# sunnyHelen/JPerceiver

Hardware: AMD Instinct MI355X
Metric: train images/sec (full train step, synthetic 3-frame batches) (higher is better)
Workload: dtype f32

## Files before the change

### include/jperceiver_hip.h

```cpp
#ifndef JPERCEIVER_HIP_H
#define JPERCEIVER_HIP_H
#include <stdint.h>

#ifdef __cplusplus
extern "C" {
#endif

int jp_conv2d_fwd(const float* x, const float* w, const float* bias, float* y, int N, int Cin, int H, int W, int Cout, int KH, int stride, int pad, int pad_mode, int act, float* ws, int ws_state, float* split_ws, const float* amax_x, float* amax_y, int* amax_y_done, float* amax_ws, float* bn_stats, int* bn_stats_parts, void* stream);
int jp_conv2d_fwd_src3(const float* x0, int c0, int up0, const float* x1, int c1, int up1, const float* x2, int c2, int up2, const float* w, const float* bias, float* y, int N, int H, int W, int Cout, int KH, int stride, int pad, int pad_mode, int act, float* ws, int ws_state, float* split_ws, const float* amax_x0, const float* amax_x1, const float* amax_x2, float* amax_y, int* amax_y_done, float* amax_ws, float* bn_stats, int* bn_stats_parts, void* stream);
int jp_conv2d_dgrad(const float* dy, const float* w, float* dx, int N, int Cin, int H, int W, int Cout, int KH, int stride, int pad, int pad_mode, int accumulate, float* ws, int ws_state, float* split_ws, const float* amax_dy, float* amax_dx, int* amax_dx_done, float* amax_ws, void* stream);
int jp_conv2d_dgrad_src3(const float* dy, const float* w, float* dx0, int c0, int up0, int acc0, float* dx1, int c1, int up1, int acc1, float* dx2, int c2, int up2, int acc2, int N, int H, int W, int Cout, int KH, int stride, int pad, int pad_mode, float* ws, int ws_state, float* split_ws, const float* amax_dy, float* amax_dx0, int* amax_dx0_done, float* amax_ws, void* stream);
long jp_conv2d_dgrad_src3_split_floats(int c0, int up0, int c1, int up1, int c2, int up2, int N, int H, int W);
int jp_conv2d_dgrad_src3_ok(int c0, int up0, int c1, int up1, int c2, int up2, int N, int H, int W, int Cout, int KH, int stride, int pad, int pad_mode);
int jp_conv2d_up_head_ok(int c0, int up0, int c1, int c2, int Cout, int KH, int stride, int pad, int pad_mode, int H, int W);
int jp_conv2d_wgrad(const float* x, const float* dy, float* dw, int N, int Cin, int H, int W, int Cout, int KH, int stride, int pad, int pad_mode, int accumulate, float* ws, long ws_floats, const float* amax_x, const float* amax_dy, float* amax_ws, void* stream);
int jp_conv2d_wgrad_src3(const float* x0, int c0, int up0, const float* x1, int c1, int up1, const float* x2, int c2, int up2, const float* dy, float* dw, int N, int H, int W, int Cout, int KH, int stride, int pad, int pad_mode, int accumulate, float* ws, long ws_floats, const float* amax_x0, const float* amax_x1, const float* amax_x2, const float* amax_dy, float* amax_ws, void* stream);
long jp_conv2d_ws_floats(int Cin, int Cout, int KH, int which);
long jp_conv2d_fwd_bn_stats_floats(int N, int OH, int OW, int Cout);
long jp_conv2d_fwd_split_floats(int N, int Cin, int H, int W, int Cout, int KH, int stride, int pad);
long jp_conv2d_dgrad_split_floats(int N, int Cin, int H, int W, int Cout, int KH, int stride, int pad);
long jp_conv2d_wgrad_ws_floats(int N, int Cin, int H, int W, int Cout, int KH, int stride, int pad);
long jp_conv2d_wgrad_src3_ws_floats(int c0, int up0, int c1, int up1, int c2, int up2, int N, int H, int W, int Cout, int KH, int stride, int pad, int pad_mode);
long jp_channel_sum_ws_floats(int N, int C, int HW);
int jp_channel_sum(const float* x, float* out, int N, int C, int HW, int accumulate, float* ws, void* stream);
int jp_pack_job_bytes(void);
int jp_pack_record_begin(void* host_jobs, int max_jobs);
int jp_pack_record_end(void);
int jp_pack_mode_is_split(int mode);
int jp_pack_replay(const void* jobs, int njobs, long total_elems, long generic_elems, void* stream);

int jp_amax_slot_floats(void);
int jp_conv2d_amax_ws_floats(void);
int jp_amax(const float* x, long n, float* out, void* stream);
int jp_amax_into(const float* x, long n, float* out, void* stream);
int jp_split_scheme(void);

long jp_bn_ws_doubles(int N, int C, int HW);
int jp_bn_train_fwd(const float* x, const float* gamma, const float* beta, const float* residual, float* y, float* running_mean, float* running_var, float* save_mean, float* save_invstd, double* ws, int N, int C, int HW, float momentum, float eps, int relu, int n_updates, float* amax_y, const float* conv_stats, int conv_parts, void* stream);
int jp_bn_train_bwd(const float* dy, const float* x, const float* y, const float* gamma, const float* beta, const float* save_mean, const float* save_invstd, float* dx, float* dres, float* dgamma, float* dbeta, double* ws, int N, int C, int HW, int relu, int acc_param_grads, float* amax_dx, void* stream);
int jp_bn_eval_fwd(const float* x, const float* gamma, const float* beta, const float* running_mean, const float* running_var, const float* residual, float* y, int N, int C, int HW, float eps, int relu, void* stream);
int jp_bn_relu_pool_fwd(const float* x, const float* gamma, const float* beta, float* pooled, uint8_t* idx, float* running_mean, float* running_var, float* save_mean, float* save_invstd, double* ws, int N, int C, int H, int W, float momentum, float eps, int n_updates, float* amax_y, void* stream);
long jp_bn_relu_pool_bwd_ws_doubles(int N, int C, int H, int W);
int jp_bn_relu_pool_bwd(const float* dpool, const uint8_t* idx, const float* x, const float* gamma, const float* beta, const float* save_mean, const float* save_invstd, float* dx, float* dgamma, float* dbeta, double* ws, int N, int C, int H, int W, int acc_param_grads, void* stream);

int jp_bn_fold_conv(const float* w, const float* conv_bias, const float* gamma, const float* beta, const float* running_mean, const float* running_var, float eps, float* w_out, float* bias_out, int Cout, int K, void* stream);
int jp_add_relu(const float* a, const float* b, float* out, long n, int relu, float* amax_out, void* stream);

int jp_maxpool_fwd(const float* x, float* y, uint8_t* idx, int NC, int H, int W, int k, int s, int p, void* stream);
int jp_maxpool_bwd(const float* dy, const uint8_t* idx, float* dx, const float* addend, int NC, int H, int W, int k, int s, int p, float* amax_dx, void* stream);
int jp_upsample2x_fwd(const float* x, float* y, int N, int C, int H, int W, int dstC, int dc0, void* stream);
int jp_upsample2x_bwd(const float* dy, float* dx, int N, int C, int H, int W, int Ctot, int c0, int accumulate, void* stream);
int jp_copy_channels(const float* src, float* dst, int N, int C, int HW, int srcC, int sc0, int dstC, int dc0, int accumulate, void* stream);
int jp_axpby(const float* a, const float* b, float* out, long n, float alpha, float beta, void* stream);
int jp_sum_n(const float* a0, const float* a1, const float* a2, const float* a3, const float* a4, float* out, long n, float* amax_out, void* stream);
int jp_mul(const float* a, const float* b, float* out, long n, float scale, void* stream);
int jp_affine(const float* a, float* out, long n, float scale, float shift, void* stream);
int jp_act_fwd(const float* x, float* y, long n, int act, void* stream);
int jp_act_bwd(const float* dy, const float* y, float* dx, long n, int act, float* amax_dx, void* stream);
long jp_act_bwd_bias_ws_floats(int N, int C, int HW);
int jp_act_bwd_bias(const float* dy, const float* y, float* dx, float* dbias, int N, int C, int HW, int act, float* amax_dx, float* bias_ws, void* stream);
int jp_mul_bcast_c(const float* a, const float* s, float* out, int N, int C, int HW, void* stream);
int jp_mul_bcast_c_bwd_s(const float* dout, const float* a, float* ds, int N, int C, int HW, void* stream);
int jp_bilinear_fwd(const float* x, float* y, int NC, int H, int W, int OH, int OW, void* stream);
int jp_bilinear_bwd(const float* dy, float* dx, int NC, int H, int W, int OH, int OW, int accumulate, void* stream);
int jp_area_downsample(const float* x, float* y, int NC, int H, int W, int f, void* stream);
int jp_fill(float* out, long n, float v, void* stream);
int jp_warp_perspective(const float* src, const float* Hm, float* dst, int B, int h, int w, int OH, int OW, void* stream);
int jp_softmax_c2(const float* x, float* y, int N, int HW, void* stream);
int jp_disp_to_depth(const float* disp, float* depth, long n, float min_depth, float max_depth, void* stream);
int jp_scale_label_assemble(const float* zwarp, const float* laywarp, const uint8_t* polymask, float* out, int B, int H, int W, int mode, void* stream);
int jp_fill_convex_poly(const int* pts, int npts, uint8_t* mask, int H, int W, void* stream);

int jp_gemm_strided_batched(const float* A, const float* B, float* C, int M, int N, int K, int lda, int ldb, int ldc, long strideA, long strideB, long strideC, int batch, int transA, int transB, float alpha, float beta, void* stream);
int jp_bias_act_rows(float* y, const float* bias, int M, int N, int act, void* stream);
int jp_colsum(const float* x, float* out, int M, int N, int accumulate, void* stream);
int jp_colmax(const float* E, float* val, int64_t* arg, int B, int R, int Cn, void* stream);
int jp_colmax_bwd(const float* dval, const int64_t* arg, float* dE, int B, int R, int Cn, void* stream);
int jp_gather_cols(const float* V, const int64_t* arg, float* T, int B, int C, int Nn, void* stream);
int jp_gather_cols_bwd(const float* dT, const int64_t* arg, float* dV, int B, int C, int Nn, void* stream);
int jp_spatial_mean(const float* x, float* out, int BC, int HW, float scale, void* stream);
int jp_spatial_mean_bwd(const float* dout, float* dx, int BC, int HW, float scale, void* stream);
int jp_bcast_matmul_fwd(const float* attn, const float* V, float* out, int B, int C, int n, void* stream);
int jp_bcast_matmul_bwd(const float* attn, const float* V, const float* dOut, float* dattn, float* dV, int B, int C, int n, void* stream);
int jp_ratio_finalize(const double* acc, float* out, double scale, void* stream);

int jp_pose_fwd(const float* axisangle, const float* translation, const float* K, float* T, float* P, int B, int invert, void* stream);
int jp_pose_bwd(const double* dP, const float* axisangle, const float* translation, const float* K, float* daxisangle, float* dtranslation, int B, int invert, int accumulate, void* stream);
int jp_cgt_warp_fwd(const float* disp, int hs, int ws, const float* invK, const float* P, const float* color, float* pred, int B, int H, int W, float min_depth, float max_depth, void* stream);
int jp_cgt_warp_bwd(const float* dpred, const float* disp, int hs, int ws, const float* invK, const float* P, const float* color, float* ddisp_up, double* dP, int B, int H, int W, float min_depth, float max_depth, int accumulate, void* stream);
int jp_ssim_l1_fwd(const float* pred, const float* target, float* out, int B, int H, int W, void* stream);
int jp_ssim_l1_bwd(const float* pred, const float* target, const int64_t* min_index, int cand, const float* gout, float gscale, float* dpred, int B, int H, int W, void* stream);
int jp_minreproj_fwd(const float* c0, const float* c1, const float* c2, const float* c3, const float* noise0, const float* noise1, int64_t* min_index, double* acc, long total, void* stream);
int jp_scalar_finalize(const double* in, float* out, int n, double scale, void* stream);
int jp_ssim_map(const float* x, const float* y, float* out, int NC, int H, int W, void* stream);
int jp_backproject(const float* depth, const float* invK, float* out, int B, int H, int W, void* stream);
int jp_project(const float* points, const float* K, const float* T, float* out, int B, int H, int W, float eps, void* stream);

int jp_row_sum(const float* x, double* out, int rows, int cols, void* stream);
int jp_smooth_fwd(const float* disp, const double* dsum, const float* img, double* acc, int B, int h, int w, void* stream);
int jp_smooth_bwd(const float* disp, const double* dsum, const float* img, const float* gout, float scale, float* g, double* gd, float* ddisp, int B, int h, int w, int accumulate, void* stream);
int jp_scale_loss_fwd(const float* disp, int hs, int ws, const float* label, double* acc, int B, int FH, int FW, float min_depth, float max_depth, int y_lo, int y_hi, int x_lo, int x_hi, void* stream);
int jp_scale_loss_bwd(const float* disp, int hs, int ws, const float* label, const double* acc, const float* gout, float scale, float* ddisp, int B, int FH, int FW, float min_depth, float max_depth, int y_lo, int y_hi, int x_lo, int x_hi, int accumulate, void* stream);
int jp_layout_loss_fwd(const float* logits, const float* label, const float* sdf, double* sums, float* loss, int B, int h, int w, float w0, float w1, float lw, float cew, float l2w, float ra, float ralpha, float rbeta, void* stream);
int jp_layout_loss_bwd(const float* logits, const float* label, const float* sdf, const double* sums, const float* gout, float* dlogits, int B, int h, int w, float w0, float w1, float lw, float cew, float l2w, float ra, float ralpha, float rbeta, int accumulate, void* stream);
int jp_sdf(const float* label, float* sdf, int* ws, int B, int h, int w, void* stream);
int jp_l1_fwd(const float* a, const float* b, double* acc, long n, void* stream);
int jp_l1_bwd(const float* a, const float* b, const float* gout, float scale, float* da, float* db, long n, void* stream);

int jp_sumsq_blocks(void);
int jp_grad_sumsq_partials(const float* g, double* partials, long n, void* stream);
int jp_sum_doubles(const double* in, double* out, int count, void* stream);
int jp_adam_clip_step(float* p, const float* g, float* m, float* v, long n, const double* normsq, float grad_scale, float max_norm, double lr, double beta1, double beta2, double eps, int step, void* stream);
int jp_adam_clip_step_dev(float* p, const float* g, float* m, float* v, long n, const double* normsq, float grad_scale, float max_norm, double beta1, double beta2, double eps, const float* state, void* stream);
int jp_rng_keep_mask(float* out, long n, uint64_t seed, float p_drop, void* stream);
int jp_rng_normal(float* out, long n, uint64_t seed, void* stream);
int jp_rng_keep_mask_dev(float* out, long n, const long* base, long offset, float p_drop, void* stream);
int jp_rng_normal_dev(float* out, long n, const long* base, long offset, void* stream);

int jp_confusion2(const float* logits, const float* gt, double* counts, int B, int HW, void* stream);
int jp_depth_eval_prepare(const float* disp_resized, const float* gt, float* pred, uint8_t* valid, int H, int W, int y0, int y1, int x0, int x1, float dmin, float dmax, void* stream);
// ... 67 lines not shown
```

### jperceiver_amd/csrc/bn.hip

```cpp
#include "jp_common.h"
#include <algorithm>

namespace {

constexpr int TPB = 256;

__global__ __launch_bounds__(TPB) void bn_stats_kernel(const float* __restrict__ x, double* __restrict__ sums,
                                                       int C, int HW, int CH, int chunk) {
    __shared__ double sm[4];
    const int c = blockIdx.x;
    const int n = blockIdx.y / CH, ck = blockIdx.y - n * CH;
    const int beg = ck * chunk, end = min(HW, beg + chunk);
    const float* xp = x + ((size_t)n * C + c) * HW;
    double s = 0.0, q = 0.0;
    float fs = 0.f, fq = 0.f;
    int run = 0;
    if (((HW | chunk) & 3) == 0) {
        const float4* x4 = reinterpret_cast<const float4*>(xp);
        for (int i = (beg >> 2) + threadIdx.x; i < (end >> 2); i += TPB) {
            const float4 v = x4[i];
            fs += (v.x + v.y) + (v.z + v.w);
            fq += (v.x * v.x + v.y * v.y) + (v.z * v.z + v.w * v.w);
            if (++run == 8) { s += fs; q += fq; fs = fq = 0.f; run = 0; }
        }
    } else {
        for (int i = beg + threadIdx.x; i < end; i += TPB) {
            const float v = xp[i];
            fs += v;
            fq += v * v;
            if (++run == 32) { s += fs; q += fq; fs = fq = 0.f; run = 0; }
        }
    }
    s += fs; q += fq;
    s = jp_block_sum_d(s, sm);
    q = jp_block_sum_d(q, sm);
    if (threadIdx.x == 0) {
        sums[(size_t)(2 * c) * gridDim.y + blockIdx.y] = s;
        sums[(size_t)(2 * c + 1) * gridDim.y + blockIdx.y] = q;
    }
}

__global__ __launch_bounds__(TPB) void bn_stats_fold_kernel(const float* __restrict__ conv_stats, double* __restrict__ sums, int parts,
                                                            int p0, int np) {
    __shared__ double sm[4];
    const int c = blockIdx.x;
    const float* a = conv_stats + ((size_t)c * 2 + 0) * parts + p0;
    const float* b = conv_stats + ((size_t)c * 2 + 1) * parts + p0;
    double s = 0.0, q = 0.0;
    for (int i = threadIdx.x; i < np; i += TPB) { s += (double)a[i]; q += (double)b[i]; }
    s = jp_block_sum_d(s, sm);
    q = jp_block_sum_d(q, sm);
    if (threadIdx.x == 0) { sums[2 * c] = s; sums[2 * c + 1] = q; }
}

__device__ __forceinline__ void bn_channel_stats(const double* __restrict__ sums, int c, int S, double count, float eps,
                                                 double* __restrict__ tot , float* mean_out, float* invstd_out,
                                                 double* var_out) {
    if (threadIdx.x < 64) {
        double a = 0.0, b = 0.0;
        for (int i = threadIdx.x; i < S; i += 64) {
            a += sums[(size_t)(2 * c) * S + i];
            b += sums[(size_t)(2 * c + 1) * S + i];
        }
        a = jp_wave_sum_d(a);
        b = jp_wave_sum_d(b);
        if (threadIdx.x == 0) { tot[0] = a; tot[1] = b; }
    }
    __syncthreads();
    const double m = tot[0] / count;
    double var = tot[1] / count - m * m;
    if (var < 0.0) var = 0.0;
    *mean_out = (float)m;
    *invstd_out = (float)(1.0 / sqrt(var + (double)eps));
    *var_out = var;
}

__device__ __forceinline__ float bn_affine(float x, float sc, float sh) { return fmaf(x, sc, sh); }
__device__ __forceinline__ float bn_shift(float beta, float mean, float sc) { return fmaf(-mean, sc, beta); }

__device__ __forceinline__ void bn_apply_body(const float* __restrict__ x, const float* __restrict__ residual,
                                              float* __restrict__ y, float sc, float sh, size_t base, int HW, int relu,
                                              unsigned* __restrict__ amax = nullptr) {
    float mx = 0.f;
    if ((HW & 3) == 0) {
        const float4* x4 = reinterpret_cast<const float4*>(x + base);
        const float4* r4 = residual ? reinterpret_cast<const float4*>(residual + base) : nullptr;
        float4* y4 = reinterpret_cast<float4*>(y + base);
        for (int i = blockIdx.x * TPB + threadIdx.x; i < (HW >> 2); i += gridDim.x * TPB) {
            const float4 a = x4[i];
            float4 v = make_float4(bn_affine(a.x, sc, sh), bn_affine(a.y, sc, sh), bn_affine(a.z, sc, sh), bn_affine(a.w, sc, sh));
            if (r4) { const float4 r = r4[i]; v.x += r.x; v.y += r.y; v.z += r.z; v.w += r.w; }
            if (relu) { v.x = fmaxf(v.x, 0.f); v.y = fmaxf(v.y, 0.f); v.z = fmaxf(v.z, 0.f); v.w = fmaxf(v.w, 0.f); }
            y4[i] = v;
            mx = fmaxf(fmaxf(mx, fmaxf(jp_fmag(v.x), jp_fmag(v.y))), fmaxf(jp_fmag(v.z), jp_fmag(v.w)));
        }
    } else {
        for (int i = blockIdx.x * TPB + threadIdx.x; i < HW; i += gridDim.x * TPB) {
            float v = bn_affine(x[base + i], sc, sh);
            if (residual) v += residual[base + i];
            if (relu) v = fmaxf(v, 0.f);
            y[base + i] = v;
            mx = fmaxf(mx, jp_fmag(v));
        }
    }
    jp_block_amax_commit(mx, amax);
}

__global__ __launch_bounds__(TPB) void bn_apply_kernel(const float* __restrict__ x, const double* __restrict__ sums,
                                                       float* __restrict__ save_mean, float* __restrict__ save_invstd,
                                                       float* __restrict__ running_mean, float* __restrict__ running_var,
                                                       const float* __restrict__ gamma,
                                                       const float* __restrict__ beta,
                                                       const float* __restrict__ residual, float* __restrict__ y,
                                                       int C, int HW, int relu, double count, float momentum, float eps,
                                                       int n_updates, int S, unsigned* __restrict__ amax) {
    __shared__ double tot[2];
    const int nc = blockIdx.y;
    const int c = nc % C;
    float mean, invstd;
    double var;
    bn_channel_stats(sums, c, S, count, eps, tot, &mean, &invstd, &var);
    if (nc < C && blockIdx.x == 0 && threadIdx.x == 0) {
        save_mean[c] = mean;
        save_invstd[c] = invstd;
        if (running_mean) {
            const float unb = (float)(count > 1.0 ? var * count / (count - 1.0) : var);
            float rm = running_mean[c], rv = running_var[c];
            for (int i = 0; i < n_updates; ++i) {
                rm = (1.f - momentum) * rm + momentum * mean;
                rv = (1.f - momentum) * rv + momentum * unb;
            }
            running_mean[c] = rm;
            running_var[c] = rv;
        }
    }
    const float sc = invstd * gamma[c];
    const float sh = bn_shift(beta[c], mean, sc);
    bn_apply_body(x, residual, y, sc, sh, (size_t)nc * HW, HW, relu, amax);
}

__global__ __launch_bounds__(TPB) void bn_eval_kernel(const float* __restrict__ x, const float* __restrict__ rm,
                                                      const float* __restrict__ rv, const float* __restrict__ gamma,
                                                      const float* __restrict__ beta,
                                                      const float* __restrict__ residual, float* __restrict__ y,
                                                      int C, int HW, float eps, int relu) {
    const int nc = blockIdx.y;
    const int c = nc % C;
    const float sc = gamma[c] / sqrtf(rv[c] + eps);
    const float sh = bn_shift(beta[c], rm[c], sc);
    bn_apply_body(x, residual, y, sc, sh, (size_t)nc * HW, HW, relu);
}

__global__ __launch_bounds__(TPB) void bn_bwd_reduce_kernel(const float* __restrict__ dy,
                                                            const float* __restrict__ x,
                                                            const float* __restrict__ y,
                                                            const float* __restrict__ mean,
                                                            const float* __restrict__ invstd,
// ... 35 lines not shown
            if (++run == 32) { s += fs; q += fq; fs = fq = 0.f; run = 0; }
        }
    }
#undef JP_BN_RED1
    s += fs; q += fq;
    s = jp_block_sum_d(s, sm);
    q = jp_block_sum_d(q, sm);
    if (threadIdx.x == 0) {
        sums[(size_t)(2 * c) * gridDim.y + blockIdx.y] = s;
        sums[(size_t)(2 * c + 1) * gridDim.y + blockIdx.y] = q;
    }
}

__global__ __launch_bounds__(TPB) void bn_bwd_apply_kernel(const float* __restrict__ dy, const float* __restrict__ x,
                                                           const float* __restrict__ y,
                                                           const float* __restrict__ mean,
                                                           const float* __restrict__ invstd,
                                                           const float* __restrict__ gamma,
                                                           const float* __restrict__ beta,
                                                           const double* __restrict__ sums, float* __restrict__ dx,
                                                           float* __restrict__ dres, float* __restrict__ dgamma,
                                                           float* __restrict__ dbeta, int C, int HW, double count,
                                                           int relu, int acc_param_grads, int S, unsigned* __restrict__ amax) {
    float mx = 0.f;
    const int nc = blockIdx.y;
    const int c = nc % C;
    const float mu = mean[c], is = invstd[c], g = gamma[c];
    const float sc = is * g, sh = bn_shift(beta[c], mu, sc);
    __shared__ double tot[2];
    if (threadIdx.x < 64) {
        double a = 0.0, b = 0.0;
        for (int i = threadIdx.x; i < S; i += 64) {
            a += sums[(size_t)(2 * c) * S + i];
            b += sums[(size_t)(2 * c + 1) * S + i];
        }
        a = jp_wave_sum_d(a);
        b = jp_wave_sum_d(b);
        if (threadIdx.x == 0) { tot[0] = a; tot[1] = b; }
    }
    __syncthreads();
    const double t1 = tot[0], t2 = tot[1];
    const float k1 = (float)(t1 / count), k2 = (float)(t2 / count);
    if (nc < C && blockIdx.x == 0 && threadIdx.x == 0) {
        const float dg = (float)t2, db = (float)t1;
        dgamma[c] = acc_param_grads ? dgamma[c] + dg : dg;
        dbeta[c] = acc_param_grads ? dbeta[c] + db : db;
    }
    const size_t base = (size_t)nc * HW;
    const float gi = g * is;
#define JP_BN_APP1(D, X, Yv, OUT, RES)                                     \
    {                                                                      \
        float d_ = (D);                                                    \
        if (relu && !((y ? (Yv) : bn_affine((X), sc, sh)) > 0.f)) d_ = 0.f; \
        RES = d_;                                                          \
        OUT = gi * (d_ - k1 - ((X) - mu) * is * k2);                       \
    }
    if ((HW & 3) == 0) {
        const float4* d4 = reinterpret_cast<const float4*>(dy + base);
        const float4* x4 = reinterpret_cast<const float4*>(x + base);
        const float4* y4 = y ? reinterpret_cast<const float4*>(y + base) : nullptr;
        float4* o4 = reinterpret_cast<float4*>(dx + base);
        float4* r4 = dres ? reinterpret_cast<float4*>(dres + base) : nullptr;
        for (int i = blockIdx.x * TPB + threadIdx.x; i < (HW >> 2); i += gridDim.x * TPB) {
            const float4 d = d4[i], a = x4[i];
            const float4 yy = y4 ? y4[i] : make_float4(0.f, 0.f, 0.f, 0.f);
            float4 o, r;
            JP_BN_APP1(d.x, a.x, yy.x, o.x, r.x) JP_BN_APP1(d.y, a.y, yy.y, o.y, r.y)
            JP_BN_APP1(d.z, a.z, yy.z, o.z, r.z) JP_BN_APP1(d.w, a.w, yy.w, o.w, r.w)
            o4[i] = o;
            mx = fmaxf(fmaxf(mx, fmaxf(jp_fmag(o.x), jp_fmag(o.y))), fmaxf(jp_fmag(o.z), jp_fmag(o.w)));
            if (r4) r4[i] = r;
        }
    } else {
        for (int i = blockIdx.x * TPB + threadIdx.x; i < HW; i += gridDim.x * TPB) {
            float o, r;
            JP_BN_APP1(dy[base + i], x[base + i], y[base + i], o, r)
            dx[base + i] = o;
            mx = fmaxf(mx, jp_fmag(o));
            if (dres) dres[base + i] = r;
        }
    }
    jp_block_amax_commit(mx, amax);
#undef JP_BN_APP1
}

__global__ __launch_bounds__(TPB) void channel_sum_kernel(const float* __restrict__ x, float* __restrict__ out,
                                                          int C, int HW, int CH, int chunk, float* __restrict__ part) {
    __shared__ double sm[4];
    const int c = blockIdx.x;
    const int n = blockIdx.y / CH, ck = blockIdx.y - n * CH;
    const int beg = ck * chunk, end = min(HW, beg + chunk);
    const float* xp = x + ((size_t)n * C + c) * HW;
    double s = 0.0;
    float fs = 0.f;
    int run = 0;
    for (int i = beg + threadIdx.x; i < end; i += TPB) {
        fs += xp[i];
        if (++run == 32) { s += fs; fs = 0.f; run = 0; }
    }
    s += fs;
    s = jp_block_sum_d(s, sm);
    if (threadIdx.x == 0) {
        if (part) part[(size_t)c * gridDim.y + blockIdx.y] = (float)s;
        else atomicAdd(&out[c], (float)s);
    }
}
__global__ void channel_fold_kernel(const float* __restrict__ part, float* __restrict__ out, int C, int S) {
    const int c = blockIdx.x * blockDim.x + threadIdx.x;
    if (c >= C) return;
    float s = 0.f;
    for (int i = 0; i < S; ++i) s += part[(size_t)c * S + i];
    out[c] += s;
}


constexpr int SP_TW = 64, SP_TH = 16;

__global__ __launch_bounds__(TPB) void bn_pool_fwd_kernel(const float* __restrict__ x, const double* __restrict__ sums,
                                                          float* __restrict__ save_mean, float* __restrict__ save_invstd,
                                                          float* __restrict__ running_mean, float* __restrict__ running_var,
                                                          const float* __restrict__ gamma, const float* __restrict__ beta,
                                                          float* __restrict__ y, uint8_t* __restrict__ idx, int C, int H, int W,
                                                          int OH, int OW, double count, float momentum, float eps, int n_updates,
                                                          int S, unsigned* __restrict__ amax) {
    constexpr int PW = (SP_TW - 1) * 2 + 3, PH = (SP_TH - 1) * 2 + 3;
    __shared__ float tile[PW * PH];
    __shared__ double tot[2];
    const int nc = blockIdx.z, c = nc % C;
    float mean, invstd;
    double var;
    bn_channel_stats(sums, c, S, count, eps, tot, &mean, &invstd, &var);
    if (nc < C && blockIdx.x == 0 && blockIdx.y == 0 && threadIdx.x == 0) {
        save_mean[c] = mean;
        save_invstd[c] = invstd;
        if (running_mean) {
            const float unb = (float)(count > 1.0 ? var * count / (count - 1.0) : var);
            float rm = running_mean[c], rv = running_var[c];
            for (int i = 0; i < n_updates; ++i) {
                rm = (1.f - momentum) * rm + momentum * mean;
                rv = (1.f - momentum) * rv + momentum * unb;
            }
            running_mean[c] = rm;
            running_var[c] = rv;
        }
    }
    const float sc = invstd * gamma[c], sh = bn_shift(beta[c], mean, sc);
    const float* xp = x + (size_t)nc * H * W;
    const int ox0 = blockIdx.x * SP_TW, oy0 = blockIdx.y * SP_TH;
    const int ix0 = ox0 * 2 - 1, iy0 = oy0 * 2 - 1;
    for (int i = threadIdx.x; i < PW * PH; i += TPB) {
        const int ly = i / PW, lx = i - ly * PW;
        const int iy = iy0 + ly, ix = ix0 + lx;
        tile[i] = ((unsigned)iy < (unsigned)H && (unsigned)ix < (unsigned)W) ? fmaxf(bn_affine(xp[iy * W + ix], sc, sh), 0.f) : -INFINITY;
    }
    __syncthreads();
    const int tx = threadIdx.x & 63, q = threadIdx.x >> 6;
    float best[4];
    int bi[4];
#pragma unroll
    for (int j = 0; j < 4; ++j) { best[j] = -INFINITY; bi[j] = 0; }
    const float* base = tile + (q * 4 * 2) * PW + tx * 2;
#pragma unroll
    for (int r = 0; r < 3 * 2 + 3; ++r) {
        float rv = base[r * PW];
        int rk = 0;
#pragma unroll
// ... 71 lines not shown
    for (int i = threadIdx.x; i < S; i += 64) {
        a += sums[(size_t)(2 * c) * S + i];
        b += sums[(size_t)(2 * c + 1) * S + i];
    }
    a = jp_wave_sum_d(a);
    b = jp_wave_sum_d(b);
    if (threadIdx.x == 0) {
        k12[2 * c] = (float)(a / count);
        k12[2 * c + 1] = (float)(b / count);
        dgamma[c] = acc_param_grads ? dgamma[c] + (float)b : (float)b;
        dbeta[c] = acc_param_grads ? dbeta[c] + (float)a : (float)a;
    }
}

__global__ __launch_bounds__(TPB) void bn_pool_bwd_apply_kernel(const float* __restrict__ dpool, const uint8_t* __restrict__ idx,
                                                                const float* __restrict__ x, const float* __restrict__ mean,
                                                                const float* __restrict__ invstd, const float* __restrict__ gamma,
                                                                const float* __restrict__ beta, const float* __restrict__ k12,
                                                                float* __restrict__ dx, long units, int C, int OH, int OW, int RB,
                                                                int bands) {
    const long u = (long)blockIdx.x * TPB + threadIdx.x;
    if (u >= units) return;
    const int OW2 = OW >> 1, W = 2 * OW;
    const int q = (int)(u % OW2);
    const long v = u / OW2;
    const int b = (int)(v % bands);
    const long nc = v / bands;
    const int c = (int)(nc % C);
    const float mu = mean[c], is = invstd[c], gm = gamma[c];
    const float sc = is * gm, sh = bn_shift(beta[c], mu, sc), gi = gm * is;
    const float k1 = k12[2 * c], k2 = k12[2 * c + 1];
    const int i0 = b * RB, i1 = min(OH, i0 + RB);
    const float* dp = dpool + nc * (long)OH * OW + 2 * q;
    const uint8_t* ip = idx + nc * (long)OH * OW + 2 * q;
    const float* xp = x + nc * 4L * OH * OW + 4 * q;
    float* op = dx + nc * 4L * OH * OW + 4 * q;
    const bool right = 2 * q + 2 < OW;
    float g[2][3];
    int k[2][3];
    auto load = [&](int slot, int i) {
        if (i < OH) {
            const float2 a = *reinterpret_cast<const float2*>(dp + (long)i * OW);
            const uchar2 cc = *reinterpret_cast<const uchar2*>(ip + (long)i * OW);
            g[slot][0] = a.x; g[slot][1] = a.y; k[slot][0] = cc.x; k[slot][1] = cc.y;
            g[slot][2] = right ? dp[(long)i * OW + 2] : 0.f;
            k[slot][2] = right ? (int)ip[(long)i * OW + 2] : -1;
        } else {
#pragma unroll
            for (int j = 0; j < 3; ++j) { g[slot][j] = 0.f; k[slot][j] = -1; }
        }
    };
    auto fin = [&](float d, float xv) {
        if (!(bn_affine(xv, sc, sh) > 0.f)) d = 0.f;
        return gi * (d - k1 - (xv - mu) * is * k2);
    };
    load(0, i0);
    for (int i = i0; i < i1; ++i) {
        load(1, i + 1);
        const float4 x0 = *reinterpret_cast<const float4*>(xp + (long)(2 * i) * W);
        const float4 x1 = *reinterpret_cast<const float4*>(xp + (long)(2 * i + 1) * W);
        float4 r0, r1;
        r0.x = k[0][0] == 4 ? g[0][0] : 0.f;
        r0.y = (k[0][0] == 5 ? g[0][0] : 0.f) + (k[0][1] == 3 ? g[0][1] : 0.f);
        r0.z = k[0][1] == 4 ? g[0][1] : 0.f;
        r0.w = (k[0][1] == 5 ? g[0][1] : 0.f) + (k[0][2] == 3 ? g[0][2] : 0.f);
        r1.x = (k[0][0] == 7 ? g[0][0] : 0.f) + (k[1][0] == 1 ? g[1][0] : 0.f);
        r1.y = (k[0][0] == 8 ? g[0][0] : 0.f) + (k[0][1] == 6 ? g[0][1] : 0.f) + (k[1][0] == 2 ? g[1][0] : 0.f) + (k[1][1] == 0 ? g[1][1] : 0.f);
        r1.z = (k[0][1] == 7 ? g[0][1] : 0.f) + (k[1][1] == 1 ? g[1][1] : 0.f);
        r1.w = (k[0][1] == 8 ? g[0][1] : 0.f) + (k[0][2] == 6 ? g[0][2] : 0.f) + (k[1][1] == 2 ? g[1][1] : 0.f) + (k[1][2] == 0 ? g[1][2] : 0.f);
        *reinterpret_cast<float4*>(op + (long)(2 * i) * W) = make_float4(fin(r0.x, x0.x), fin(r0.y, x0.y), fin(r0.z, x0.z), fin(r0.w, x0.w));
        *reinterpret_cast<float4*>(op + (long)(2 * i + 1) * W) = make_float4(fin(r1.x, x1.x), fin(r1.y, x1.y), fin(r1.z, x1.z), fin(r1.w, x1.w));
#pragma unroll
        for (int j = 0; j < 3; ++j) { g[0][j] = g[1][j]; k[0][j] = k[1][j]; }
    }
}

void chunking(int N, int C, int HW, int* CH, int* chunk) {
    int ch = std::max(1, 2048 / std::max(1, N * C));
    ch = std::min(ch, std::max(1, HW / 2048));
    *chunk = (HW + ch - 1) / ch;
    *CH = (HW + *chunk - 1) / *chunk;
}

}

extern "C" long jp_bn_ws_doubles(int N, int C, int HW) {
    int CH, chunk;
    chunking(N, C, HW, &CH, &chunk);
    return 2L * C * N * CH;
}

extern "C" int jp_bn_train_fwd(const float* x, const float* gamma, const float* beta, const float* residual,
                               float* y, float* running_mean, float* running_var, float* save_mean,
                               float* save_invstd, double* ws, int N, int C, int HW, float momentum, float eps,
                               int relu, int n_updates, float* amax_y, const float* conv_stats, int conv_parts, void* stream) {
    JP_CHECK_ARG(x && gamma && beta && y && save_mean && save_invstd && ws, "bn_train_fwd: null pointer");
    JP_CHECK_ARG(N > 0 && C > 0 && HW > 0, "bn_train_fwd: bad dims");
    hipStream_t st = (hipStream_t)stream;
    int CH, chunk;
    chunking(N, C, HW, &CH, &chunk);
    int S = N * CH;
    if (conv_stats && conv_parts > 0) {
        hipLaunchKernelGGL(bn_stats_fold_kernel, dim3(C), dim3(TPB), 0, st, conv_stats, ws, conv_parts, 0, conv_parts);
        S = 1;
    } else {
        hipLaunchKernelGGL(bn_stats_kernel, dim3(C, N * CH), dim3(TPB), 0, st, x, ws, C, HW, CH, chunk);
    }
    const int gx = std::min(jp_cdiv(HW, 4 * TPB), 64);
    hipLaunchKernelGGL(bn_apply_kernel, dim3(gx, N * C), dim3(TPB), 0, st, x, ws, save_mean, save_invstd, running_mean,
                       running_var, gamma, beta, residual, y, C, HW, relu, (double)N * HW, momentum, eps, n_updates, S,
                       reinterpret_cast<unsigned*>(amax_y));
    JP_LAUNCH_CHECK();
}

extern "C" int jp_bn_train_bwd(const float* dy, const float* x, const float* y, const float* gamma, const float* beta,
                               const float* save_mean, const float* save_invstd, float* dx, float* dres,
                               float* dgamma, float* dbeta, double* ws, int N, int C, int HW, int relu,
                               int acc_param_grads, float* amax_dx, void* stream) {
    JP_CHECK_ARG(dy && x && gamma && beta && save_mean && save_invstd && dx && dgamma && dbeta && ws, "bn_train_bwd: null pointer");
    hipStream_t st = (hipStream_t)stream;
    int CH, chunk;
    chunking(N, C, HW, &CH, &chunk);
    hipLaunchKernelGGL(bn_bwd_reduce_kernel, dim3(C, N * CH), dim3(TPB), 0, st, dy, x, y, save_mean, save_invstd, gamma,
                       beta, ws, C, HW, CH, chunk, relu);
    const int gx = std::min(jp_cdiv(HW, 4 * TPB), 64);
    hipLaunchKernelGGL(bn_bwd_apply_kernel, dim3(gx, N * C), dim3(TPB), 0, st, dy, x, y, save_mean, save_invstd, gamma,
                       beta, ws, dx, dres, dgamma, dbeta, C, HW, (double)N * HW, relu, acc_param_grads, N * CH,
                       reinterpret_cast<unsigned*>(amax_dx));
    JP_LAUNCH_CHECK();
}

extern "C" int jp_bn_relu_pool_fwd(const float* x, const float* gamma, const float* beta, float* pooled, uint8_t* idx,
                                   float* running_mean, float* running_var, float* save_mean, float* save_invstd, double* ws,
                                   int N, int C, int H, int W, float momentum, float eps, int n_updates, float* amax_y,
                                   void* stream) {
    JP_CHECK_ARG(x && gamma && beta && pooled && idx && save_mean && save_invstd && ws, "bn_relu_pool_fwd: null pointer");
    JP_CHECK_ARG(N > 0 && C > 0 && H >= 4 && W >= 4 && H % 4 == 0 && W % 4 == 0, "bn_relu_pool_fwd: H and W must be multiples of 4");
    hipStream_t st = (hipStream_t)stream;
    const int HW = H * W, OH = H / 2, OW = W / 2;
    int CH, chunk;
    chunking(N, C, HW, &CH, &chunk);
    hipLaunchKernelGGL(bn_stats_kernel, dim3(C, N * CH), dim3(TPB), 0, st, x, ws, C, HW, CH, chunk);
    hipLaunchKernelGGL(bn_pool_fwd_kernel, dim3(jp_cdiv(OW, SP_TW), jp_cdiv(OH, SP_TH), N * C), dim3(TPB), 0, st, x, ws, save_mean,
                       save_invstd, running_mean, running_var, gamma, beta, pooled, idx, C, H, W, OH, OW, (double)N * HW, momentum,
                       eps, n_updates, N * CH, reinterpret_cast<unsigned*>(amax_y));
    JP_LAUNCH_CHECK();
}

extern "C" long jp_bn_relu_pool_bwd_ws_doubles(int N, int C, int H, int W) {
    return jp_bn_ws_doubles(N, C, (H / 2) * (W / 2)) + C;
}
extern "C" int jp_bn_relu_pool_bwd(const float* dpool, const uint8_t* idx, const float* x, const float* gamma, const float* beta,
                                   const float* save_mean, const float* save_invstd, float* dx, float* dgamma, float* dbeta,
                                   double* ws, int N, int C, int H, int W, int acc_param_grads, void* stream) {
    JP_CHECK_ARG(dpool && idx && x && gamma && beta && save_mean && save_invstd && dx && dgamma && dbeta && ws,
                 "bn_relu_pool_bwd: null pointer");
    JP_CHECK_ARG(N > 0 && C > 0 && H >= 4 && W >= 4 && H % 4 == 0 && W % 4 == 0, "bn_relu_pool_bwd: H and W must be multiples of 4");
    hipStream_t st = (hipStream_t)stream;
    const int OH = H / 2, OW = W / 2;
    int CH, chunk;
    chunking(N, C, OH * OW, &CH, &chunk);
    float* k12 = reinterpret_cast<float*>(ws + 2L * C * N * CH);
    hipLaunchKernelGGL(bn_pool_bwd_reduce_kernel, dim3(C, N * CH), dim3(TPB), 0, st, dpool, idx, x, save_mean, save_invstd, gamma, beta,
                       ws, C, H, W, OH, OW, CH, chunk);
    hipLaunchKernelGGL(bn_pool_bwd_fold_kernel, dim3(C), dim3(64), 0, st, ws, k12, dgamma, dbeta, N * CH, (double)N * H * W,
                       acc_param_grads);
    const int RB = OH >= 128 ? 32 : 8, bands = jp_cdiv(OH, RB);
    const long units = (long)N * C * bands * (OW / 2);
    hipLaunchKernelGGL(bn_pool_bwd_apply_kernel, dim3((unsigned)jp_cdiv(units, (long)TPB)), dim3(TPB), 0, st, dpool, idx, x, save_mean,
                       save_invstd, gamma, beta, k12, dx, units, C, OH, OW, RB, bands);
    JP_LAUNCH_CHECK();
}

extern "C" long jp_channel_sum_ws_floats(int N, int C, int HW) {
    int CH, chunk;
    chunking(N, C, HW, &CH, &chunk);
    return (long)C * N * CH;
}
extern "C" int jp_channel_sum(const float* x, float* out, int N, int C, int HW, int accumulate, float* ws, void* stream) {
    JP_CHECK_ARG(x && out && N > 0 && C > 0 && HW > 0, "channel_sum: bad args");
    hipStream_t st = (hipStream_t)stream;
    if (!accumulate) JP_HIP(hipMemsetAsync(out, 0, sizeof(float) * C, st));
    int CH, chunk;
    chunking(N, C, HW, &CH, &chunk);
    hipLaunchKernelGGL(channel_sum_kernel, dim3(C, N * CH), dim3(TPB), 0, st, x, out, C, HW, CH, chunk, ws);
    if (ws) hipLaunchKernelGGL(channel_fold_kernel, dim3(jp_cdiv(C, 64)), dim3(64), 0, st, ws, out, C, N * CH);
    JP_LAUNCH_CHECK();
}

extern "C" int jp_bn_eval_fwd(const float* x, const float* gamma, const float* beta, const float* running_mean,
                              const float* running_var, const float* residual, float* y, int N, int C, int HW,
                              float eps, int relu, void* stream) {
    JP_CHECK_ARG(x && gamma && beta && running_mean && running_var && y && N > 0 && C > 0 && HW > 0, "bn_eval_fwd: bad args");
    hipStream_t st = (hipStream_t)stream;
    const int gx = std::min(jp_cdiv(HW, 4 * TPB), 64);
    jp_prof_before("jp_bn_eval_fwd", 0.0, st);
    hipLaunchKernelGGL(bn_eval_kernel, dim3(gx, N * C), dim3(TPB), 0, st, x, running_mean, running_var, gamma, beta,
                       residual, y, C, HW, eps, relu);
    jp_prof_after(st);
    JP_LAUNCH_CHECK();
}
```

Baseline: 128.2.

## Add single-pass on-chip BatchNorm kernels holding each channel slab in registers

When N*HW per channel fits in one workgroup's registers, BN forward, backward and the stats pass for bn-relu-pool run as a single kernel per channel. Each kernel loads the slab once, reduces in-block and applies, replacing the separate reduce and apply launches and the second global read. The cost is only C workgroups per launch, which gives low parallelism on small-channel layers, plus heavy register use from 32 floats per thread. JP_LAUNCH_CHECK is assumed to return, so the old path is skipped.

```diff
diff --git a/include/jperceiver_hip.h b/include/jperceiver_hip.h
--- a/include/jperceiver_hip.h
+++ b/include/jperceiver_hip.h
@@ -36,6 +36,7 @@
 int jp_split_scheme(void);
 
 long jp_bn_ws_doubles(int N, int C, int HW);
+int jp_bn_onchip(int N, int C, int HW, int* max_slab);
 int jp_bn_train_fwd(const float* x, const float* gamma, const float* beta, const float* residual, float* y, float* running_mean, float* running_var, float* save_mean, float* save_invstd, double* ws, int N, int C, int HW, float momentum, float eps, int relu, int n_updates, float* amax_y, const float* conv_stats, int conv_parts, void* stream);
 int jp_bn_train_bwd(const float* dy, const float* x, const float* y, const float* gamma, const float* beta, const float* save_mean, const float* save_invstd, float* dx, float* dres, float* dgamma, float* dbeta, double* ws, int N, int C, int HW, int relu, int acc_param_grads, float* amax_dx, void* stream);
 int jp_bn_eval_fwd(const float* x, const float* gamma, const float* beta, const float* running_mean, const float* running_var, const float* residual, float* y, int N, int C, int HW, float eps, int relu, void* stream);
diff --git a/jperceiver_amd/csrc/bn.hip b/jperceiver_amd/csrc/bn.hip
--- a/jperceiver_amd/csrc/bn.hip
+++ b/jperceiver_amd/csrc/bn.hip
@@ -53,6 +53,16 @@
     if (threadIdx.x == 0) { sums[2 * c] = s; sums[2 * c + 1] = q; }
 }
 
+__device__ __forceinline__ void bn_finish_stats(double s, double q, double count, float eps, float* mean_out, float* invstd_out,
+                                                double* var_out) {
+    const double m = s / count;
+    double var = q / count - m * m;
+    if (var < 0.0) var = 0.0;
+    *mean_out = (float)m;
+    *invstd_out = (float)(1.0 / sqrt(var + (double)eps));
+    *var_out = var;
+}
+
 __device__ __forceinline__ void bn_channel_stats(const double* __restrict__ sums, int c, int S, double count, float eps,
                                                  double* __restrict__ tot , float* mean_out, float* invstd_out,
                                                  double* var_out) {
@@ -67,12 +77,7 @@
         if (threadIdx.x == 0) { tot[0] = a; tot[1] = b; }
     }
     __syncthreads();
-    const double m = tot[0] / count;
-    double var = tot[1] / count - m * m;
-    if (var < 0.0) var = 0.0;
-    *mean_out = (float)m;
-    *invstd_out = (float)(1.0 / sqrt(var + (double)eps));
-    *var_out = var;
+    bn_finish_stats(tot[0], tot[1], count, eps, mean_out, invstd_out, var_out);
 }
 
 __device__ __forceinline__ float bn_affine(float x, float sc, float sh) { return fmaf(x, sc, sh); }
@@ -274,6 +279,213 @@
     }
     jp_block_amax_commit(mx, amax);
 #undef JP_BN_APP1
+}
+
+constexpr int OC_TPB = 1024, OC_PER = 32, OC_TPB_SMALL = 256;
+#ifndef JP_BN_ONCHIP_MAX
+#define JP_BN_ONCHIP_MAX (OC_TPB * OC_PER)
+#endif
+static_assert(JP_BN_ONCHIP_MAX <= OC_TPB * OC_PER, "the on-chip slab must fit the workgroup's registers");
+
+struct OcSlab {
+    int c, C, HW, per, nu;
+    unsigned long long magic;
+    template <int T>
+    __device__ __forceinline__ bool live(int k) const { return k * T < nu; }
+    template <int T>
+    __device__ __forceinline__ bool has(int k) const { return k * T + (int)threadIdx.x < nu; }
+    template <int T, bool VEC>
+    __device__ __forceinline__ size_t off(int k) const {
+        const unsigned u = k * T + threadIdx.x;
+        const unsigned n = (unsigned)((u * magic) >> 32), i = u - n * per;
+        return ((size_t)n * C + c) * HW + (VEC ? 4 * i : i);
+    }
+};
+template <int T, bool VEC>
+__device__ __forceinline__ void oc_load(const float* __restrict__ p, const OcSlab& sl, float (&v)[OC_PER]) {
+#pragma unroll
+    for (int k = 0; k < OC_PER; ++k) v[k] = 0.f;
+    if (VEC) {
+#pragma unroll
+        for (int k = 0; k < OC_PER / 4; ++k) {
+            if (!sl.live<T>(k)) break;
+            if (sl.has<T>(k)) {
+                const float4 a = *reinterpret_cast<const float4*>(p + sl.off<T, true>(k));
+                v[4 * k] = a.x; v[4 * k + 1] = a.y; v[4 * k + 2] = a.z; v[4 * k + 3] = a.w;
+            }
+        }
+    } else {
+#pragma unroll
+        for (int k = 0; k < OC_PER; ++k) {
+            if (!sl.live<T>(k)) break;
+            if (sl.has<T>(k)) v[k] = p[sl.off<T, false>(k)];
+        }
+    }
+}
+template <int T, bool VEC>
+__device__ __forceinline__ void oc_store(float* __restrict__ p, const OcSlab& sl, const float (&v)[OC_PER]) {
+    if (VEC) {
+#pragma unroll
+        for (int k = 0; k < OC_PER / 4; ++k) {
+            if (!sl.live<T>(k)) break;
+            if (sl.has<T>(k)) *reinterpret_cast<float4*>(p + sl.off<T, true>(k)) = make_float4(v[4 * k], v[4 * k + 1], v[4 * k + 2], v[4 * k + 3]);
+        }
+    } else {
+#pragma unroll
+        for (int k = 0; k < OC_PER; ++k) {
+            if (!sl.live<T>(k)) break;
+            if (sl.has<T>(k)) p[sl.off<T, false>(k)] = v[k];
+        }
+    }
+}
+template <int T, bool VEC>
+__device__ __forceinline__ float oc_amax(const OcSlab& sl, const float (&v)[OC_PER]) {
+    float mx = 0.f;
+#pragma unroll
+    for (int k = 0; k < OC_PER; ++k) {
+        if (!sl.live<T>(VEC ? k >> 2 : k)) break;
+        if (sl.has<T>(VEC ? k >> 2 : k)) mx = fmaxf(mx, jp_fmag(v[k]));
+    }
+    return mx;
+}
+template <int T>
+__device__ __forceinline__ void oc_block_sum2(double& a, double& b, double* sm ) {
+    a = jp_wave_sum_d(a);
+    b = jp_wave_sum_d(b);
+    if ((threadIdx.x & 63) == 0) { sm[2 * (threadIdx.x >> 6)] = a; sm[2 * (threadIdx.x >> 6) + 1] = b; }
+    __syncthreads();
+    a = b = 0.0;
+#pragma unroll
+    for (int i = 0; i < T / 64; ++i) { a += sm[2 * i]; b += sm[2 * i + 1]; }
+}
+
+__device__ __forceinline__ void oc_sum_sq(const float (&v)[OC_PER], double& s, double& q) {
+#pragma unroll
+    for (int k = 0; k < OC_PER; k += 4) {
+        s += (double)((v[k] + v[k + 1]) + (v[k + 2] + v[k + 3]));
+        q += (double)((v[k] * v[k] + v[k + 1] * v[k + 1]) + (v[k + 2] * v[k + 2] + v[k + 3] * v[k + 3]));
+    }
+}
+
+template <int T, bool VEC>
+__global__ __launch_bounds__(T) void bn_onchip_stats_kernel(const float* __restrict__ x, double* __restrict__ sums, OcSlab sl) {
+    __shared__ double sm[2 * T / 64];
+    sl.c = blockIdx.x;
+    const int c = sl.c;
+    float v[OC_PER];
+    oc_load<T, VEC>(x, sl, v);
+    double s = 0.0, q = 0.0;
+    oc_sum_sq(v, s, q);
+    oc_block_sum2<T>(s, q, sm);
+    if (threadIdx.x == 0) { sums[2 * c] = s; sums[2 * c + 1] = q; }
+}
+
+template <int T, bool VEC>
+__global__ __launch_bounds__(T) void bn_onchip_fwd_kernel(const float* __restrict__ x, const float* __restrict__ conv_stats,
+                                                               int parts, float* __restrict__ save_mean,
+                                                               float* __restrict__ save_invstd, float* __restrict__ running_mean,
+                                                               float* __restrict__ running_var, const float* __restrict__ gamma,
+                                                               const float* __restrict__ beta, const float* __restrict__ residual,
+                                                               float* __restrict__ y, OcSlab sl, int relu, double count,
+                                                               float momentum, float eps, int n_updates, unsigned* __restrict__ amax) {
+    __shared__ double sm[2 * T / 64];
+    sl.c = blockIdx.x;
+    const int c = sl.c;
+    float v[OC_PER], r[OC_PER];
+    oc_load<T, VEC>(x, sl, v);
+    if (residual) oc_load<T, VEC>(residual, sl, r);
+    double s = 0.0, q = 0.0;
+    if (conv_stats) {
+        const float* a = conv_stats + ((size_t)c * 2 + 0) * parts;
+        const float* b = conv_stats + ((size_t)c * 2 + 1) * parts;
+        for (int i = threadIdx.x; i < parts; i += T) { s += (double)a[i]; q += (double)b[i]; }
+    } else {
+        oc_sum_sq(v, s, q);
+    }
+    oc_block_sum2<T>(s, q, sm);
+    float mean, invstd;
+    double var;
+    bn_finish_stats(s, q, count, eps, &mean, &invstd, &var);
+    if (threadIdx.x == 0) {
+        save_mean[c] = mean;
+        save_invstd[c] = invstd;
+        if (running_mean) {
+            const float unb = (float)(count > 1.0 ? var * count / (count - 1.0) : var);
+            float rm = running_mean[c], rv = running_var[c];
+            for (int i = 0; i < n_updates; ++i) {
+                rm = (1.f - momentum) * rm + momentum * mean;
+                rv = (1.f - momentum) * rv + momentum * unb;
+            }
+            running_mean[c] = rm;
+            running_var[c] = rv;
+        }
+    }
+    const float sc = invstd * gamma[c];
+    const float sh = bn_shift(beta[c], mean, sc);
+    float mx = 0.f;
+#pragma unroll
+    for (int k = 0; k < OC_PER; ++k) {
+        float o = bn_affine(v[k], sc, sh);
+        if (residual) o += r[k];
+        if (relu) o = fmaxf(o, 0.f);
+        v[k] = o;
+    }
+    oc_store<T, VEC>(y, sl, v);
+    if (amax) mx = oc_amax<T, VEC>(sl, v);
+    jp_block_amax_commit(mx, amax);
+}
+
+template <int T, bool VEC>
+__global__ __launch_bounds__(T) void bn_onchip_bwd_kernel(const float* __restrict__ dy, const float* __restrict__ x,
+                                                               const float* __restrict__ y, const float* __restrict__ mean,
+                                                               const float* __restrict__ invstd, const float* __restrict__ gamma,
+                                                               const float* __restrict__ beta, float* __restrict__ dx,
+                                                               float* __restrict__ dres, float* __restrict__ dgamma,
+                                                               float* __restrict__ dbeta, OcSlab sl, double count,
+                                                               int relu, int acc_param_grads, unsigned* __restrict__ amax) {
+    __shared__ double sm[2 * T / 64];
+    sl.c = blockIdx.x;
+    const int c = sl.c;
+    const float mu = mean[c], is = invstd[c], g = gamma[c];
+    const float sc = is * g, sh = bn_shift(beta[c], mu, sc), gi = g * is;
+    float d[OC_PER], a[OC_PER];
+    oc_load<T, VEC>(dy, sl, d);
+    oc_load<T, VEC>(x, sl, a);
+    if (relu) {
+        if (y) {
+            float yy[OC_PER];
+            oc_load<T, VEC>(y, sl, yy);
+#pragma unroll
+            for (int k = 0; k < OC_PER; ++k)
+                if (!(yy[k] > 0.f)) d[k] = 0.f;
+        } else {
+#pragma unroll
+            for (int k = 0; k < OC_PER; ++k)
+                if (!(bn_affine(a[k], sc, sh) > 0.f)) d[k] = 0.f;
+        }
+    }
+    double s = 0.0, q = 0.0;
+#pragma unroll
+    for (int k = 0; k < OC_PER; k += 4) {
+        float t[4];
+#pragma unroll
+        for (int j = 0; j < 4; ++j) t[j] = d[k + j] * (a[k + j] - mu) * is;
+        s += (double)((d[k] + d[k + 1]) + (d[k + 2] + d[k + 3]));
+        q += (double)((t[0] + t[1]) + (t[2] + t[3]));
+    }
+    oc_block_sum2<T>(s, q, sm);
+    const float k1 = (float)(s / count), k2 = (float)(q / count);
+    if (threadIdx.x == 0) {
+        const float dg = (float)q, db = (float)s;
+        dgamma[c] = acc_param_grads ? dgamma[c] + dg : dg;
+        dbeta[c] = acc_param_grads ? dbeta[c] + db : db;
+    }
+    if (dres) oc_store<T, VEC>(dres, sl, d);
+#pragma unroll
+    for (int k = 0; k < OC_PER; ++k) a[k] = gi * (d[k] - k1 - (a[k] - mu) * is * k2);
+    oc_store<T, VEC>(dx, sl, a);
+    const float mx = amax ? oc_amax<T, VEC>(sl, a) : 0.f;
+    jp_block_amax_commit(mx, amax);
 }
 
 __global__ __launch_bounds__(TPB) void channel_sum_kernel(const float* __restrict__ x, float* __restrict__ out,
@@ -511,6 +723,18 @@
     *CH = (HW + *chunk - 1) / *chunk;
 }
 
+bool bn_onchip(int N, int HW) { return (long)N * HW <= (long)JP_BN_ONCHIP_MAX; }
+OcSlab oc_slab(int N, int C, int HW) {
+    const int per = (HW & 3) == 0 ? HW >> 2 : HW;
+    return OcSlab{0, C, HW, per, N * per, (0x100000000ULL + per - 1) / per};
+}
+bool bn_onchip_small(int N, int HW) { return (long)N * HW <= (long)OC_TPB_SMALL * OC_PER; }
+
+}
+
+extern "C" int jp_bn_onchip(int N, int C, int HW, int* max_slab) {
+    if (max_slab) *max_slab = JP_BN_ONCHIP_MAX;
+    return (N > 0 && C > 0 && HW > 0 && bn_onchip(N, HW)) ? 1 : 0;
 }
 
 extern "C" long jp_bn_ws_doubles(int N, int C, int HW) {
@@ -526,6 +750,16 @@
     JP_CHECK_ARG(x && gamma && beta && y && save_mean && save_invstd && ws, "bn_train_fwd: null pointer");
     JP_CHECK_ARG(N > 0 && C > 0 && HW > 0, "bn_train_fwd: bad dims");
     hipStream_t st = (hipStream_t)stream;
+    if (bn_onchip(N, HW)) {
+        const float* cs = (conv_stats && conv_parts > 0) ? conv_stats : nullptr;
+        const bool small = bn_onchip_small(N, HW), vec = (HW & 3) == 0;
+        auto k = small ? (vec ? bn_onchip_fwd_kernel<OC_TPB_SMALL, true> : bn_onchip_fwd_kernel<OC_TPB_SMALL, false>)
+                       : (vec ? bn_onchip_fwd_kernel<OC_TPB, true> : bn_onchip_fwd_kernel<OC_TPB, false>);
+        hipLaunchKernelGGL(k, dim3(C), dim3(small ? OC_TPB_SMALL : OC_TPB), 0, st, x, cs, conv_parts, save_mean, save_invstd, running_mean, running_var, gamma,
+                           beta, residual, y, oc_slab(N, C, HW), relu, (double)N * HW, momentum, eps, n_updates,
+                           reinterpret_cast<unsigned*>(amax_y));
+        JP_LAUNCH_CHECK();
+    }
     int CH, chunk;
     chunking(N, C, HW, &CH, &chunk);
     int S = N * CH;
@@ -547,7 +781,16 @@
                                float* dgamma, float* dbeta, double* ws, int N, int C, int HW, int relu,
                                int acc_param_grads, float* amax_dx, void* stream) {
     JP_CHECK_ARG(dy && x && gamma && beta && save_mean && save_invstd && dx && dgamma && dbeta && ws, "bn_train_bwd: null pointer");
+    JP_CHECK_ARG(N > 0 && C > 0 && HW > 0, "bn_train_bwd: bad dims");
     hipStream_t st = (hipStream_t)stream;
+    if (bn_onchip(N, HW)) {
+        const bool small = bn_onchip_small(N, HW), vec = (HW & 3) == 0;
+        auto k = small ? (vec ? bn_onchip_bwd_kernel<OC_TPB_SMALL, true> : bn_onchip_bwd_kernel<OC_TPB_SMALL, false>)
+                       : (vec ? bn_onchip_bwd_kernel<OC_TPB, true> : bn_onchip_bwd_kernel<OC_TPB, false>);
+        hipLaunchKernelGGL(k, dim3(C), dim3(small ? OC_TPB_SMALL : OC_TPB), 0, st, dy, x, y, save_mean, save_invstd, gamma, beta, dx, dres, dgamma, dbeta, oc_slab(N, C, HW),
+                           (double)N * HW, relu, acc_param_grads, reinterpret_cast<unsigned*>(amax_dx));
+        JP_LAUNCH_CHECK();
+    }
     int CH, chunk;
     chunking(N, C, HW, &CH, &chunk);
     hipLaunchKernelGGL(bn_bwd_reduce_kernel, dim3(C, N * CH), dim3(TPB), 0, st, dy, x, y, save_mean, save_invstd, gamma,
@@ -569,10 +812,17 @@
     const int HW = H * W, OH = H / 2, OW = W / 2;
     int CH, chunk;
     chunking(N, C, HW, &CH, &chunk);
-    hipLaunchKernelGGL(bn_stats_kernel, dim3(C, N * CH), dim3(TPB), 0, st, x, ws, C, HW, CH, chunk);
+    int S = N * CH;
+    if (bn_onchip(N, HW)) {
+        if (bn_onchip_small(N, HW)) hipLaunchKernelGGL((bn_onchip_stats_kernel<OC_TPB_SMALL, true>), dim3(C), dim3(OC_TPB_SMALL), 0, st, x, ws, oc_slab(N, C, HW));
+        else hipLaunchKernelGGL((bn_onchip_stats_kernel<OC_TPB, true>), dim3(C), dim3(OC_TPB), 0, st, x, ws, oc_slab(N, C, HW));
+        S = 1;
+    } else {
+        hipLaunchKernelGGL(bn_stats_kernel, dim3(C, N * CH), dim3(TPB), 0, st, x, ws, C, HW, CH, chunk);
+    }
     hipLaunchKernelGGL(bn_pool_fwd_kernel, dim3(jp_cdiv(OW, SP_TW), jp_cdiv(OH, SP_TH), N * C), dim3(TPB), 0, st, x, ws, save_mean,
                        save_invstd, running_mean, running_var, gamma, beta, pooled, idx, C, H, W, OH, OW, (double)N * HW, momentum,
-                       eps, n_updates, N * CH, reinterpret_cast<unsigned*>(amax_y));
+                       eps, n_updates, S, reinterpret_cast<unsigned*>(amax_y));
     JP_LAUNCH_CHECK();
 }
 
```

After: 127.7. No clear change (-0.4%).
